# CederGroupHub/sparse-lm

Measured on AMD Instinct MI355X. Metric: fits/sec over 50-alpha Lasso path at n=100k p=5k, higher is better.
Workload: dtype f64

## Files before the change

include/slm_engine.h:

```cpp
#ifndef SLM_ENGINE_H
#define SLM_ENGINE_H

#include <stddef.h>
#include <stdint.h>

#ifdef __cplusplus
extern "C" {
#endif

#define SLM_ABI_VERSION 22

typedef enum slm_status {
  SLM_OK = 0,
  SLM_ERR_BAD_ARG = 1,
  SLM_ERR_OOM = 2,
  SLM_ERR_HIP = 3,
  SLM_ERR_NO_DEVICE = 4,
  SLM_ERR_COMM = 5,
  SLM_ERR_NOT_CONVERGED = 6,
  SLM_ERR_NON_FINITE = 7,
  SLM_ERR_UNSUPPORTED = 8
} slm_status;

typedef struct slm_engine slm_engine;
typedef struct slm_dataset slm_dataset;
// ... 186 lines not shown
int slm_solve_constrained(slm_dataset* ds, const double* a, const double* A, int32_t m, const double* lo, const double* hi,
                          const slm_solve_opts* opts, double tol_inner, int32_t max_sweeps, const double* beta0, int32_t warm,
                          double* beta_out, double* lambda_out, slm_point_info* info);

int slm_dataset_covariance(slm_dataset* ds, const double* row_weight, int64_t n_eff);
int slm_dataset_covariance_folds(slm_dataset* ds, const double* const* row_weights, const int64_t* n_effs, int32_t count);
int slm_dataset_covariance_folds_begin(slm_dataset* ds, const double* const* row_weights, const int64_t* n_effs, int32_t count,
                                       int32_t* started_out);
int slm_dataset_covariance_folds_finish(slm_dataset* ds);
int slm_dataset_covariance_count(slm_dataset* ds, int32_t* count_out);
int slm_dataset_covariance_clear(slm_dataset* ds);
int slm_dataset_covariance_download(slm_dataset* ds, int32_t index, double* G_out, double* c_out, double scalars_out[4]);

int slm_dataset_read_ceiling(slm_dataset* ds, int32_t reps, double* gbs_out, double* ms_out);

int slm_dataset_model_gram(slm_dataset* ds, double* G_out);
int slm_dataset_set_replicated(slm_dataset* ds, int32_t replicated);

#define SLM_COMM_ID_BYTES 128
int slm_comm_unique_id(uint8_t id_out[SLM_COMM_ID_BYTES]);
int slm_comm_init(slm_engine* eng, int32_t rank, int32_t n_ranks,
                  const uint8_t id[SLM_COMM_ID_BYTES]);
int slm_comm_info(slm_engine* eng, int32_t* rank_out, int32_t* n_ranks_out);
int slm_comm_collectives(slm_engine* eng, int64_t* count_out);
int slm_comm_all_reduce_probe(slm_engine* eng, int64_t count, int32_t reps, double* us_out);
int slm_comm_init_local(slm_engine** engines, int32_t n_ranks, double timeout_s);
int slm_dataset_set_global_rows(slm_dataset* ds, int64_t n_global);
int slm_comm_destroy(slm_engine* eng);

#ifdef __cplusplus
// ... 4 lines not shown
```

sparse-lm_amd/csrc/data_kernels.hpp:

```cpp
#pragma once
#include <hip/hip_runtime.h>
#include <stdint.h>

#include "grad_kernel.hpp"
#include "tail_kernels.hpp"

namespace slm {

static __global__ __launch_bounds__(256) void transpose_f2c_kernel(const double* __restrict__ src, int64_t n,
                                                            int64_t p, double* __restrict__ dst,
                                                            int64_t ld) {
  __shared__ double tile[32][33];
  const int tx = threadIdx.x & 31, ty = threadIdx.x >> 5;
  const int64_t i0 = (int64_t)blockIdx.x * 32, j0 = (int64_t)blockIdx.y * 32;
  for (int k = ty; k < 32; k += 8) {
    const int64_t i = i0 + tx, j = j0 + k;
    tile[k][tx] = (i < n && j < p) ? src[j * n + i] : 0.0;
  }
  __syncthreads();
  for (int k = ty; k < 32; k += 8) {
    const int64_t i = i0 + k, j = j0 + tx;
    if (i < n && j < p) dst[i * ld + j] = tile[tx][k];
  }
}

static __global__ __launch_bounds__(256) void tile_columns_kernel(const double* __restrict__ X, int64_t n, int64_t ld,
                                                           double* __restrict__ XT) {
  __shared__ double tile[32][33];
  const int tx = threadIdx.x & 31, ty = threadIdx.x >> 5;
  const int64_t i0 = (int64_t)blockIdx.x * 32, j0 = (int64_t)blockIdx.y * 32;
  for (int k = ty; k < 32; k += 8) {
    const int64_t i = i0 + k, j = j0 + tx;
    tile[k][tx] = (i < n && j < ld) ? X[i * ld + j] : 0.0;
  }
  __syncthreads();
  for (int k = ty; k < 32; k += 8) {
    const int64_t j = j0 + k;
    if (j < ld) XT[((int64_t)blockIdx.x * ld + j) * 32 + tx] = tile[tx][k];
  }
}

template <int U, bool NT, bool RR = false>
__global__ __launch_bounds__(256) void read_stream_kernel(const double* __restrict__ src, int64_t count2 ,
                                                          double* __restrict__ sink) {
  const d2* p = reinterpret_cast<const d2*>(src);
  const int64_t per = (count2 + gridDim.x - 1) / gridDim.x;
  const int64_t lo = RR ? (int64_t)blockIdx.x * (U * 256) : (int64_t)blockIdx.x * per;
  const int64_t hi = RR ? count2 : (lo + per < count2 ? lo + per : count2);
  const int64_t step = RR ? (int64_t)gridDim.x * (U * 256) : (int64_t)U * 256;
  double a0 = 0.0, a1 = 0.0;
  int64_t i = lo + threadIdx.x;
  for (; i + (int64_t)(U - 1) * 256 < hi; i += step) {
    d2 v[U];
#pragma unroll
// ... 199 lines not shown
```

sparse-lm_amd/csrc/engine.hip:

```cpp
#include "engine_internal.hpp"

static thread_local std::string g_last_error;

int fail(int code, const char* fmt, ...) {
  char buf[1024];
  va_list ap;
  va_start(ap, fmt);
  vsnprintf(buf, sizeof(buf), fmt, ap);
  va_end(ap);
  g_last_error = buf;
  return code;
}

RcclApi g_rccl;

int load_rccl() {
  if (g_rccl.lib) return SLM_OK;
  const char* names[] = {"librccl.so.1", "librccl.so", "/opt/rocm/lib/librccl.so.1"};
  void* lib = nullptr;
  for (const char* nm : names) {
    lib = dlopen(nm, RTLD_NOW | RTLD_GLOBAL);
    if (lib) break;
  }
  if (!lib) return fail(SLM_ERR_COMM, "cannot load librccl: %s", dlerror());
// ... 239 lines not shown
}

static void dataset_free(slm_dataset* ds) {
  if (!ds) return;
  dfree(ds->X); dfree(ds->y); dfree(ds->rw); dfree(ds->yzero); dfree(ds->rw_lanes); dfree(ds->rvec);
  dfree(ds->order); dfree(ds->gid); dfree(ds->gstart);
  dfree(ds->partial); dfree(ds->loss_partial); dfree(ds->R);
  dfree(ds->g); dfree(ds->z); dfree(ds->beta); dfree(ds->zprev); dfree(ds->gprev);
  dfree(ds->u); dfree(ds->gscale); dfree(ds->a0); dfree(ds->b0); dfree(ds->d0);
  dfree(ds->lambda); dfree(ds->dctl);
  dfree(ds->pts); dfree(ds->betas_out); dfree(ds->gn_out); dfree(ds->infos);
  dfree(ds->ws_idx); dfree(ds->ws_pos); dfree(ds->ws_gs); dfree(ds->ws_gl);
  dfree(ds->ws_score); dfree(ds->ws_XW); dfree(ds->ws_part); dfree(ds->ws_G); dfree(ds->ws_Gx); dfree(ds->XT); dfree(ds->ws_owner);
  dfree(ds->ws_nt); dfree(ds->stop_words); dfree(ds->sse_Z); dfree(ds->sse_part); dfree(ds->split_state);
  dfree(ds->cons_state); dfree(ds->cons_buf);
  dfree(ds->colnorm); dfree(ds->lt_dR); dfree(ds->lt_d2); dfree(ds->lt_part); dfree(ds->lt_cols); dfree(ds->lt_stamp);
  cov_pending_drop(ds);
  ds->cov.clear();
  ds->cov_all_hold.reset();
  ds->cov_all = nullptr;
  dfree(ds->cov_Z); dfree(ds->cov_fp); dfree(ds->cov_partial);
  mg_free(ds);
  if (ds->h_split) (void)hipHostFree(ds->h_split);
  if (ds->hctl) (void)hipHostFree(ds->hctl);
  if (ds->h_small_out) (void)hipHostFree(ds->h_small_out);
  if (ds->h_vec) (void)hipHostFree(ds->h_vec);
  if (ds->h_stage) (void)hipHostFree(ds->h_stage);
  if (ds->h_pts) (void)hipHostFree(ds->h_pts);
  for (auto& e : ds->ev)
    if (e) (void)hipEventDestroy(e);
// ... 561 lines not shown
```

sparse-lm_amd/csrc/engine_internal.hpp:

```cpp
#pragma once
#include <hip/hip_runtime.h>

#include <dlfcn.h>
#include <stdarg.h>
#include <stdio.h>
#include <stdlib.h>
#include <string.h>

#include <algorithm>
#include <cmath>
#include <chrono>
#include <condition_variable>
#include <memory>
#include <mutex>
#include <numeric>
#include <string>
#include <vector>

#include "../../include/slm_engine.h"
#include "host_logic.hpp"
#include "data_kernels.hpp"
#include "grad_kernel.hpp"
#include "tail_kernels.hpp"
#include "ws_kernels.hpp"
// ... 182 lines not shown
  double* cov_Z = nullptr;
  double* cov_partial = nullptr;
  int cov_partial_sets = 0;
  size_t partial_elems = 0;
  double* cov_fp = nullptr;
  double* split_state = nullptr;
  double* h_split = nullptr;
  double* cons_state = nullptr;
  double* cons_buf = nullptr;
  size_t cons_buf_doubles = 0;
  double* stop_words = nullptr;
  double* XT = nullptr;
  bool XT_ready = false, XT_failed = false;
  double* colnorm = nullptr;
  bool colnorm_ready = false;
  double *lt_dR = nullptr, *lt_d2 = nullptr, *lt_part = nullptr;
  int32_t *lt_cols = nullptr, *lt_stamp = nullptr;
  struct MgEntry {
    float* G = nullptr;
    double fp1 = 0.0, fp2 = 0.0, n_eff = 0.0;
    bool own = false;
  };
  std::vector<MgEntry> mg;
  double* mg_vec = nullptr;
  double* mg_Z = nullptr;
  bool mg_failed = false;
  double mg_build_ms = 0.0;
  int ws_sets = 0;
  const GradKernel* gk[SLM_MAX_LANES] = {};
  int nblk[SLM_MAX_LANES] = {};
// ... 54 lines not shown

struct LaneSetup {
  int B = 1;
  const double* rw = nullptr;
  int64_t rw_stride = 0;
  double n_eff[SLM_MAX_CELLS] = {};
};
LaneSetup default_lanes(slm_dataset* ds, int B);
int enqueue_gradient(slm_dataset* ds, const LaneSetup& ls, const double* y, const int* done, hipEvent_t ev_start, hipEvent_t ev_stop,
                     int64_t n_rows = 0, const int* skip = nullptr, GradNames* names = nullptr);
int enqueue_gradient_split(const slm_host::Knobs& kn, slm_dataset* ds, const LaneSetup& ls, const double* y, const int* done, const PathCtl* ctl, const WsArgs* wa,
                           hipEvent_t ev_start, hipEvent_t ev_stop, int64_t n_rows = 0, bool unit_bracket = false, const int* skip = nullptr,
                           GradNames* names = nullptr);
bool split_usable(const slm_host::Knobs& kn, slm_dataset* ds);
int ensure_xt(const slm_host::Knobs& kn, slm_dataset* ds);
int check_launch();
void launch_rowdot(const slm_host::Knobs& kn, slm_dataset* ds, const SplitKernel* sk, int nblk, int B, SplitArgs& a, hipStream_t s,
                  const char** name = nullptr);
int enqueue_gradient_cov(slm_dataset* ds, int B, const int* entry_of, const int* done, hipEvent_t ev_start, hipEvent_t ev_stop,
                         const PathCtl* ctl = nullptr, const WsArgs* wa = nullptr, GradNames* names = nullptr);
void launch_tail(const TailArgs& ta, hipStream_t s);
int64_t sketch_rows(int64_t n);
int power_iteration(const slm_host::Knobs& kn, slm_dataset* ds, const LaneSetup& ls_in, double* L_out , int iters, int64_t n_rows = 0);
int estimate_lipschitz(const slm_host::Knobs& kn, slm_dataset* ds, double* L_out, int iters);
int allow_big_lds(const void* fn, int device);
static const int kProfStride = 3;
static const int kPowerItersSolve = 2;
int cov_fingerprints(slm_dataset* ds, const double* const* w, int count, double* out );
int cov_find(const slm_dataset* ds, double fp1, double fp2, double n_eff);
void cov_pending_drop(slm_dataset* ds);
// ... 9 lines not shown
```

sparse-lm_amd/csrc/engine_path.hip:

```cpp
#include "engine_internal.hpp"

static int ws_policy(const slm_host::Knobs& kn, const slm_dataset* ds, uint32_t flags) {
  if (ds->max_group > WS_KCAP / 2 || ds->n < 4) return 0;
  if (kn.ws == 0 || (flags & SLM_FLAG_NO_WORKING_SET)) return 0;
  const bool big = (double)ds->n * (double)ds->ld >= 67108864.0;
  return (big || (flags & SLM_FLAG_WORKING_SET) || kn.ws == 1) ? 2 : 1;
}

static bool small_ok(const slm_host::Knobs& kn, const slm_dataset* ds, uint32_t flags) {
  if (!(flags & SLM_FLAG_ON_CHIP)) return false;
  if (flags & (SLM_FLAG_NO_RESTART | SLM_FLAG_PROFILE | SLM_FLAG_FISTA_ONLY | SLM_FLAG_WORKING_SET | SLM_FLAG_NO_WORKING_SET))
    return false;
  if (!kn.on_chip) return false;
  return ds->p <= SM_PMAX && (double)ds->n * (double)ds->ld <= 131072.0 && !row_sharded(ds);
}
static bool split_possible(const slm_dataset* ds) {
  return ds->sk != nullptr && (ds->sk->rowdot != nullptr || !ds->XT_failed);
}
static int max_lanes_for(const slm_host::Knobs& kn, const slm_dataset* ds, uint32_t flags) {
  if (small_ok(kn, ds, flags)) return ds->lane_cap;
  if ((ws_policy(kn, ds, flags) == 2 || (double)ds->n * (double)ds->ld >= 67108864.0) && split_possible(ds)) {
    if (ws_policy(kn, ds, flags) == 2 && !row_sharded(ds) && ds->sk->rowdot != nullptr && !ds->XT_failed)
      return kMaxLanes;
    return SPLIT_LANES;
// ... 908 lines not shown
    for (int l = 0; l < B; ++l) {
      int64_t mine = lanes[l].n_points;
      if (shared_path && interleave) mine = slm_host::interleaved_points(slm_host::LaneWalk{h[l].pt_lo, h[l].n_points, h[l].stride, h[l].tail_pt});
      most = std::max<int64_t>(most, mine);
    }
    expected = 1 + most;
    planned_end = expected;
  }
  {
    bool cold = true;
    for (int l = 0; l < B; ++l) cold = cold && lanes[l].beta0 == nullptr;
    if (cold && shared_path && use_ws && !ws_late && !sharded && !cov_on && split && !any_rw && !ds->rw &&
        !custom_scale && expected > 0 && o.max_iter >= 4 && !(o.flags & SLM_FLAG_FISTA_ONLY) && kn.sample_start) {
      const int64_t least = kn.sample_min_rows;
      if (n >= least) n_sample = n / kn.sample_div;
    }
  }
  mg_forced = kn.mg == 2;
  mg_cap = slm_host::model_gram_cap(ld, 3.0e9, kMgEntries);
  mg_ok = use_ws && split && (big_x || mg_forced) && !sharded && !cov_on && !(o.flags & SLM_FLAG_NO_MODEL_GRAM) &&
                     (size_t)ds->lane_cap >= (size_t)kMaxLanes && ws_n_sets <= mg_cap && mg_possible(kn, ds);
  if (mg_ok && mg_forced) expected = 0;
  if (mg_ok && !mg_forced && !ds->mg.empty()) {
    bool all = ws_n_sets > 0;
    for (int st = 0; st < ws_n_sets && all; ++st) {
      const int l = ws_set_lane[st];
      all = lanes[l].row_weight == nullptr;
      const double ne = ls.n_eff[l] > 0 ? ls.n_eff[l] : (double)ds->n_global;
      bool have = false;
      for (const auto& e : ds->mg) have = have || (e.own && e.n_eff == ne);
// ... 643 lines not shown
```

sparse-lm_amd/csrc/engine_solve.hip:

```cpp
#include "engine_internal.hpp"

#define SLM_GK(W, C, R, B) {W, C, R, B, 0, grad_fused_kernel<W, C, R, B>, "grad_fused_kernel<" #W "," #C "," #R "," #B ">"}
#define SLM_RK(W, C, B, D) {W, C, 1, B, D, grad_ring_kernel<W, C, B, D>, "grad_ring_kernel<" #W "," #C "," #B "," #D ">"}
static const GradKernel kGradRing[] = {
    SLM_RK(8, 1, 1, 3), SLM_RK(8, 2, 1, 3), SLM_RK(8, 3, 1, 3), SLM_RK(8, 4, 1, 3), SLM_RK(8, 5, 1, 2),
    SLM_RK(8, 1, 2, 3), SLM_RK(8, 2, 2, 3), SLM_RK(8, 3, 2, 3), SLM_RK(8, 4, 2, 3), SLM_RK(8, 5, 2, 2),
    SLM_RK(8, 1, 3, 3), SLM_RK(8, 2, 3, 3), SLM_RK(8, 3, 3, 3), SLM_RK(8, 4, 3, 3), SLM_RK(8, 5, 3, 2),
    SLM_RK(8, 1, 4, 3), SLM_RK(8, 2, 4, 3), SLM_RK(8, 3, 4, 3), SLM_RK(8, 4, 4, 3), SLM_RK(8, 5, 4, 2),
    SLM_RK(8, 1, 5, 3), SLM_RK(8, 2, 5, 3), SLM_RK(8, 3, 5, 3), SLM_RK(8, 4, 5, 3),
    SLM_RK(8, 1, 6, 3), SLM_RK(8, 2, 6, 3), SLM_RK(8, 3, 6, 3),
};
static const GradKernel kGradDefault[] = {
    SLM_GK(1, 1, 4, 1), SLM_GK(2, 1, 4, 1), SLM_GK(4, 1, 4, 1), SLM_GK(8, 1, 4, 1), SLM_GK(8, 2, 4, 1),
    SLM_GK(8, 3, 4, 1), SLM_GK(8, 4, 2, 1), SLM_GK(8, 5, 2, 1), SLM_GK(8, 6, 2, 1), SLM_GK(8, 8, 2, 1),
    SLM_GK(8, 10, 1, 1),
    SLM_GK(1, 1, 4, 2), SLM_GK(2, 1, 4, 2), SLM_GK(4, 1, 4, 2), SLM_GK(8, 1, 4, 2), SLM_GK(8, 2, 4, 2),
    SLM_GK(8, 3, 4, 2), SLM_GK(8, 4, 2, 2), SLM_GK(8, 5, 2, 2), SLM_GK(8, 6, 2, 2), SLM_GK(8, 8, 1, 2),
    SLM_GK(1, 1, 4, 3), SLM_GK(2, 1, 4, 3), SLM_GK(4, 1, 4, 3), SLM_GK(8, 1, 4, 3), SLM_GK(8, 2, 4, 3),
    SLM_GK(8, 3, 4, 3), SLM_GK(8, 4, 2, 3), SLM_GK(8, 5, 2, 3), SLM_GK(8, 6, 1, 3),
    SLM_GK(1, 1, 4, 4), SLM_GK(2, 1, 4, 4), SLM_GK(4, 1, 4, 4), SLM_GK(8, 1, 4, 4), SLM_GK(8, 2, 4, 4),
    SLM_GK(8, 3, 2, 4), SLM_GK(8, 4, 2, 4), SLM_GK(8, 5, 1, 4),
};
static const GradKernel kGradExtra[] = {
    SLM_GK(8, 5, 1, 1), SLM_GK(8, 5, 3, 1), SLM_GK(8, 5, 4, 1), SLM_GK(8, 4, 4, 1), SLM_GK(8, 6, 1, 1),
// ... 16 lines not shown
  return &kSplitAnyWidth;
}

int xtr_max_row_blocks(int cus, int64_t ld) {
  return slm_host::xtr_row_blocks_most(cus, ld, XTR_CB);
}
int launch_xtr(const slm_host::Knobs& kn, int cus, SplitArgs& a, hipStream_t s, bool sample, const char** name) {
  double per_cu = kn.xtr_wgs_per_cu;
  const bool wide = a.lane_slots > SPLIT_LANES;
  if (wide) per_cu = 1.0;
  const slm_host::XtrGrid g = slm_host::xtr_grid(a.n, a.ld, XTR_CB, (int64_t)(xtr_max_row_blocks(cus, a.ld) * per_cu / 2.0));
  const int xb = g.xb, yb = g.yb;
  a.xrows = g.rows;
  const int extra = wide ? a.n_lanes - SPLIT_LANES : 0;
  const char* nm;
  if (wide && extra >= 1 && extra <= 2) {
    if (sample) { hipLaunchKernelGGL(xtr18_sample_kernel, dim3(xb, yb), dim3(XTR_WAVES * 64), 0, s, a); nm = "xtr18_sample_kernel"; }
    else { hipLaunchKernelGGL(xtr18_mfma_kernel, dim3(xb, yb), dim3(XTR_WAVES * 64), 0, s, a); nm = "xtr18_mfma_kernel"; }
  } else if (wide && extra >= 3 && extra <= 4) {
    if (sample) { hipLaunchKernelGGL(xtr20_sample_kernel, dim3(xb, yb), dim3(XTR_WAVES * 64), 0, s, a); nm = "xtr20_sample_kernel"; }
    else { hipLaunchKernelGGL(xtr20_mfma_kernel, dim3(xb, yb), dim3(XTR_WAVES * 64), 0, s, a); nm = "xtr20_mfma_kernel"; }
  } else if (wide) {
    if (sample) { hipLaunchKernelGGL(xtr32_sample_kernel, dim3(xb, yb), dim3(XTR_WAVES * 64), 0, s, a); nm = "xtr32_sample_kernel"; }
    else { hipLaunchKernelGGL(xtr32_mfma_kernel, dim3(xb, yb), dim3(XTR_WAVES * 64), 0, s, a); nm = "xtr32_mfma_kernel"; }
  } else {
    if (sample) { hipLaunchKernelGGL(xtr_sample_kernel, dim3(xb, yb), dim3(XTR_WAVES * 64), 0, s, a); nm = "xtr_sample_kernel"; }
    else { hipLaunchKernelGGL(xtr_mfma_kernel, dim3(xb, yb), dim3(XTR_WAVES * 64), 0, s, a); nm = "xtr_mfma_kernel"; }
  }
  if (name) *name = nm;
  return yb;
}
// ... 148 lines not shown
  const int64_t nr = n_rows > 0 ? n_rows : ds->n;
  a.n = nr; a.ld = ds->ld; a.rows_base = nr / nblk; a.rows_rem = nr % nblk;
  a.p2 = (int)(ds->ld / 2);
  a.n_lanes = ls.B;
  const bool unit = ev_start != nullptr && unit_bracket;
  if (unit) HIP_TRY(hipEventRecord(ev_start, s));
  launch_rowdot(kn, ds, sk, nblk, ls.B, a, s, names ? &names->resid : nullptr);
  if (wa && ctl) {
    const char* nm;
    if (kn.resid_vec && halves == 1) { hipLaunchKernelGGL(sk->resid, dim3(nblk), dim3(256), 0, s, a); nm = "resid_ws_kernel<16>"; }
    else if (halves == 2) { hipLaunchKernelGGL(resid32_mfma_kernel, dim3(nblk, 1), dim3(RM_WAVES * 64), 0, s, a); nm = "resid32_mfma_kernel"; }
    else { hipLaunchKernelGGL(resid_mfma_kernel, dim3(nblk, halves), dim3(RM_WAVES * 64), 0, s, a); nm = "resid_mfma_kernel"; }
    if (names) names->ws_resid = nm;
  }
  if (ev_start && !unit) HIP_TRY(hipEventRecord(ev_start, s));
  const int xblk = launch_xtr(kn, ds->eng->cus, a, s, n_rows > 0 && ctl != nullptr,
                              names ? &names->product : nullptr);
  if (ev_stop) HIP_TRY(hipEventRecord(ev_stop, s));
  ReduceArgs ra;
  ra.partial = ds->partial;
  ra.loss_partial = ds->loss_partial;
  ra.g = ds->g;
  ra.done = done;
  ra.nblk = xblk;
  ra.nblk_loss = nblk;
  ra.skip = skip;
  ra.n_lanes = a.lane_slots;
  ra.ld = ds->ld;
  for (int l = 0; l < kMaxLanes; ++l) {
    const double ne = ls.n_eff[l] > 0 ? ls.n_eff[l] : (double)ds->n_global;
    ra.scale[l] = 1.0 / ne;
    ra.loss_scale[l] = 0.5 / ne;
// ... 180 lines not shown
  HIP_TRY(hipMemsetAsync(ds->z, 0, sizeof(double) * ld, s));
  LaneSetup ls = default_lanes(ds, 1);
  ls.n_eff[0] = sums[0];
  SLM_TRY(enqueue_gradient(ds, ls, ds->yzero, nullptr, nullptr, nullptr));
  HIP_TRY(hipMemsetAsync(ds->yzero, 0, sizeof(double) * n, s));
  const int cblocks = ds->eng->cus * 8;
  hipLaunchKernelGGL(center_kernel, dim3(cblocks), dim3(256), 0, s, ds->X, ds->y, n, p, ld, ds->g, ymean);
  SLM_TRY(check_launch());
  if (x_mean_out) HIP_TRY(hipMemcpyAsync(x_mean_out, ds->g, sizeof(double) * p, hipMemcpyDeviceToHost, s));
  HIP_TRY(hipStreamSynchronize(s));
  if (y_mean_out) *y_mean_out = ymean;
  ds->L_valid = false;
  ds->sketch_valid = false;
  ds->carry_valid = false;
  ds->XT_ready = false;
  mg_invalidate(ds);
  return SLM_OK;
}

template <typename Launch>
static int timed_launches(hipStream_t s, int reps, double* ms_out, Launch launch) {
  hipEvent_t e0, e1;
  HIP_TRY(hipEventCreate(&e0));
  HIP_TRY(hipEventCreate(&e1));
  HIP_TRY(hipEventRecord(e0, s));
  int rc = SLM_OK;
  for (int r = 0; r < reps && rc == SLM_OK; ++r) rc = launch();
  HIP_TRY(hipEventRecord(e1, s));
  HIP_TRY(hipEventSynchronize(e1));
  float ms = 0.f;
// ... 295 lines not shown
    ds->XT_ready = true;
    ds->colnorm_ready = false;
    const dim3 grid((unsigned)row_tiles, (unsigned)((ld + 31) / 32));
    hipLaunchKernelGGL(tile_columns_kernel, grid, dim3(256), 0, s, (const double*)ds->X, n, ld, ds->XT);
  }
  if (ds->XT && ds->XT_ready && !ds->colnorm_ready && !ds->rw && !row_sharded(ds) && kn.light_pass) {
    if (!ds->colnorm && pool_malloc((void**)&ds->colnorm, sizeof(double) * (size_t)ld) != hipSuccess) {
      (void)hipGetLastError();
      ds->colnorm = nullptr;
    }
    if (ds->colnorm) {
      hipLaunchKernelGGL(colnorm_kernel, dim3((unsigned)((ld + 7) / 8)), dim3(256), 0, s, (const double*)ds->XT, n, ld, 1.0 / (double)ds->n_global,
                         ds->colnorm);
      ds->colnorm_ready = true;
    }
  }
  return SLM_OK;
}

extern "C" int slm_eval_sse_sparse(slm_dataset* ds, const int32_t* cols, int32_t n_cols, const double* Zs,
                                   int32_t m, const double* row_weight, double* sse_out) {
  if (!ds || !cols || !Zs || !sse_out) return fail(SLM_ERR_BAD_ARG, "NULL argument");
  if (m <= 0 || n_cols <= 0) return fail(SLM_ERR_BAD_ARG, "m and n_cols must be positive");
  if (n_cols > WS_KCAP) return fail(SLM_ERR_UNSUPPORTED, "more than %d columns: use slm_eval_sse", WS_KCAP);
  for (int k = 0; k < n_cols; ++k)
    if (cols[k] < 0 || cols[k] >= ds->p) return fail(SLM_ERR_BAD_ARG, "cols[%d] = %d outside [0, p)", k, cols[k]);
  slm_engine* eng = ds->eng;
  HIP_TRY(hipSetDevice(eng->device));
  hipStream_t s = eng->stream;
  const int64_t n = ds->n;
// ... 279 lines not shown
```

sparse-lm_amd/csrc/host_logic.hpp:

```cpp
#pragma once
#include <stddef.h>
#include <math.h>
#include <stdint.h>
#include <stdio.h>
#include <stdlib.h>

#include <algorithm>
#include <utility>
#include <vector>

#if defined(__HIPCC__)
#define SLM_HD __host__ __device__
#else
#define SLM_HD
#endif

namespace slm_host {

struct PoolLedger {
  struct Idle { int dev; size_t bytes; void* block; };
  struct Live { void* block; int dev; size_t bytes; };
  std::vector<Idle> idle;
  std::vector<Live> live;
  size_t idle_bytes = 0;
// ... 197 lines not shown
  bool carry = true;
  bool ws_carry = true;
  bool eval_fused = false;
  double ws_theta = 0.85;
  int ws_append = 48;
  int ws_kinit = 0;
  int ws_bb = 1;
  int ws_one_solver = 0;
  bool hard_callwide = false;
  int ws_miss_factor = 4;
  int ws_miss_div = 8;
  double ws_fill = 0.0;
  bool sample_start = true;
  int64_t sample_min_rows = 65536;
  int sample_div = 4;
  int mg = -1;
  bool handover = true;
  bool light_pass = true;
  bool lag_handover = true;
  bool gram_owner = true;
  double device_pool_gb = -1.0;
  bool allow_any_arch = false;
  int trace = 0;
  bool trace_poll = false;

  template <typename Get>
  static Knobs from(Get get) {
    Knobs k;
    auto text = [&](const char* name) -> const char* { return get(name); };
    auto is_set = [&](const char* name) { return text(name) != nullptr; };
// ... 26 lines not shown
    if (const char* e = text("SLM_WS_THETA")) {
      const double v = atof(e);
      if (v > 0.0 && v <= 1.0) k.ws_theta = v;
    }
    as_int("SLM_WS_APPEND", 1, 512, &k.ws_append);
    as_int("SLM_WS_KINIT", 16, 512, &k.ws_kinit);
    if (const char* e = text("SLM_WS_BB")) k.ws_bb = atoi(e) != 0;
    if (const char* e = text("SLM_WS_ONE_SOLVER")) k.ws_one_solver = atoi(e) != 0;
    k.hard_callwide = is_set("SLM_HARD_CALLWIDE");
    as_int("SLM_WS_MISS_FACTOR", 1, 8, &k.ws_miss_factor);
    as_int("SLM_WS_MISS_DIV", 1, 4096, &k.ws_miss_div);
    if (const char* e = text("SLM_WS_FILL")) k.ws_fill = std::max(0.1, std::min(1.0, atof(e)));
    k.sample_start = !is_set("SLM_NO_SAMPLE_START");
    if (const char* e = text("SLM_SAMPLE_START_MIN_ROWS")) k.sample_min_rows = std::max<int64_t>(64, atoll(e));
    as_int("SLM_SAMPLE_DIV", 1, 64, &k.sample_div);
    if (const char c = first("SLM_MG")) k.mg = c == '0' ? 0 : (c == '2' ? 2 : -1);
    k.handover = !is_set("SLM_NO_HANDOVER");
    k.light_pass = !is_set("SLM_NO_LIGHT_PASS");
    k.gram_owner = !is_set("SLM_NO_GRAM_OWNER");
    k.lag_handover = !is_set("SLM_NO_LAG_HANDOVER");
    if (const char* e = text("SLM_DEVICE_POOL_GB")) k.device_pool_gb = std::max(0.0, atof(e));
    k.allow_any_arch = is_set("SLM_ALLOW_ANY_ARCH");
    if (const char c = first("SLM_TRACE")) k.trace = (c >= '1' && c <= '3') ? c - '0' : 1;
    k.trace_poll = is_set("SLM_TRACE_POLL");
    return k;
  }
};

}
```

sparse-lm_amd/csrc/split_kernels.hpp:

```cpp
#pragma once
#include <hip/hip_runtime.h>
#include <stdint.h>

#include "grad_kernel.hpp"
#include "tail_kernels.hpp"
#include "ws_kernels.hpp"

namespace slm {

constexpr int SPLIT_LANES = 16;
constexpr int SPLIT_RSTRIDE = 16;
constexpr int SPLIT_HALVES = SLM_MAX_LANES / SPLIT_LANES;
static_assert(SLM_MAX_LANES % SPLIT_LANES == 0 && SPLIT_HALVES >= 1 && SPLIT_HALVES <= 2, "one or two halves of sixteen lanes");
constexpr int ROWDOT_LANES = 5;

struct SplitArgs {
  const double* X;
  const double* y;
  const double* rw;
  int64_t rw_stride;
  const double* z;
  double* R;
  double* partial;
  double* loss_partial;
  const int* done;
  const PathCtl* ctl;
  const double* XW;
  const int32_t* idx;
  const WsCtl* ws;
  int64_t n, ld, rows_base, rows_rem;
  int p2;
  int n_lanes;
  int lane0;
  int xrows;
  int xrows_ws;
  const double* XT;
  int lane_slots;
  int64_t r_plane;
  const int* skip;
};
__device__ __forceinline__ bool split_off(const SplitArgs& a) {
  return (a.done != nullptr && *a.done != 0) || (a.skip != nullptr && *a.skip != 0);
}
__device__ __forceinline__ int split_slots(const SplitArgs& a) { return a.lane_slots > 0 ? a.lane_slots : SPLIT_LANES; }

__device__ __forceinline__ void split_masks(const SplitArgs& a, unsigned& live, unsigned& on_ws, int half = 0) {
  const int l = threadIdx.x & 63;
  const int L = SPLIT_LANES * half + l;
  int lv = 0, sp = 0;
  if (l < SPLIT_LANES && L < a.n_lanes) {
    if (a.ctl == nullptr) {
      lv = 1;
    } else {
      const int dn = a.ctl[L].done, id = a.ctl[L].idle, zs = a.ctl[L].zsup;
// ... 411 lines not shown
            if (col < ld) out[col] = acc[h][2 * c + e][r];
          }
    }
  }
}

static __global__ __launch_bounds__(XTR_WAVES * 64, 2) void xtr_mfma_kernel(SplitArgs a) { xtr_mfma_body<1>(a); }
static __global__ __launch_bounds__(XTR_WAVES * 64, 1) void xtr32_mfma_kernel(SplitArgs a) { xtr_mfma_body<2>(a); }
static __global__ __launch_bounds__(XTR_WAVES * 64, 2) void xtr_sample_kernel(SplitArgs a) { xtr_mfma_body<1>(a); }
static __global__ __launch_bounds__(XTR_WAVES * 64, 1) void xtr32_sample_kernel(SplitArgs a) { xtr_mfma_body<2>(a); }
static __global__ __launch_bounds__(XTR_WAVES * 64, 1) void xtr18_mfma_kernel(SplitArgs a) { xtr_mfma_body<1, 2>(a); }
static __global__ __launch_bounds__(XTR_WAVES * 64, 1) void xtr20_mfma_kernel(SplitArgs a) { xtr_mfma_body<1, 4>(a); }
static __global__ __launch_bounds__(XTR_WAVES * 64, 1) void xtr18_sample_kernel(SplitArgs a) { xtr_mfma_body<1, 2>(a); }
static __global__ __launch_bounds__(XTR_WAVES * 64, 1) void xtr20_sample_kernel(SplitArgs a) { xtr_mfma_body<1, 4>(a); }

constexpr int XZ_WAVES = 4;
constexpr int XZ_T = 4;

template <int NT, int H, int E = 0>
__device__ __forceinline__ void rowdot_step(const double* xt0, int64_t ld, const double* const (&zp)[H],
                                            const double* const (&zpe)[E > 0 ? E : 1], int g_n, double* mine, double* pe) {
  constexpr int EE = E > 0 ? E : 1;
  slm_d4 acc[H][NT][2];
#pragma unroll
  for (int h = 0; h < H; ++h)
#pragma unroll
    for (int t = 0; t < NT; ++t) acc[h][t][0] = acc[h][t][1] = slm_d4{0.0, 0.0, 0.0, 0.0};
  d2 ex[EE][NT];
#pragma unroll
  for (int e = 0; e < EE; ++e)
// ... 414 lines not shown
```

sparse-lm_amd/sparselm_amd/_engine.py:

```python

from __future__ import annotations

import ctypes as C
import os
import sys
import threading
import weakref

import numpy as np

_LIB_NAME = "libslm_hip.so"
_LIB_DIR = os.path.join(os.path.dirname(os.path.abspath(__file__)), "_lib")

SLM_OK = 0
SLM_ERR_BAD_ARG = 1
SLM_ERR_OOM = 2
SLM_ERR_HIP = 3
SLM_ERR_NO_DEVICE = 4
SLM_ERR_COMM = 5
SLM_ERR_NOT_CONVERGED = 6
SLM_ERR_NON_FINITE = 7
SLM_ERR_UNSUPPORTED = 8

FLAG_NO_RESTART = 1
FLAG_PROFILE = 2
FLAG_COLD_START = 4
FLAG_FRESH_L = 8
FLAG_FISTA_ONLY = 16
FLAG_WORKING_SET = 32
FLAG_NO_WORKING_SET = 64
FLAG_ON_CHIP = 128
FLAG_COVARIANCE = 256
FLAG_PROFILE_UNIT = 1024
FLAG_NO_MODEL_GRAM = 512

COMM_ID_BYTES = 128
ABI_VERSION = 22

ABI_SYMBOLS = (
    "slm_abi_version",
    "slm_last_error",
    "slm_device_count",
    "slm_host_alloc",
    "slm_host_free",
    "slm_engine_create",
    "slm_engine_destroy",
    "slm_engine_synchronize",
    "slm_reload_knobs",
    "slm_engine_device_info",
    "slm_dataset_create",
    "slm_dataset_create_device",
    "slm_dataset_create_synthetic",
# ... 19 lines not shown
    "slm_solve_path",
    "slm_solve_lanes",
    "slm_solve_lanes_reweighted",
    "slm_solve_path_lanes",
    "slm_solve_standardized_sgl",
    "slm_solve_constrained",
    "slm_dataset_covariance",
    "slm_dataset_covariance_folds",
    "slm_dataset_covariance_folds_begin",
    "slm_dataset_covariance_folds_finish",
    "slm_dataset_covariance_count",
    "slm_dataset_covariance_clear",
    "slm_dataset_covariance_download",
    "slm_dataset_model_gram",
    "slm_dataset_read_ceiling",
    "slm_dataset_set_replicated",
    "slm_comm_unique_id",
    "slm_comm_init",
    "slm_comm_info",
    "slm_comm_collectives",
    "slm_comm_all_reduce_probe",
    "slm_comm_init_local",
    "slm_dataset_set_global_rows",
    "slm_comm_destroy",
)


class EngineError(RuntimeError):
    """HIP / RCCL / device failure reported by the engine."""

# ... 202 lines not shown
            "slm_solve_lanes_reweighted": [vp, P(_Lane), P(_Reweight), i32, P(_SolveOpts), P(_SolveStats), P(i32)],
            "slm_solve_path_lanes": [
                vp, P(_PenaltyStruct), P(_PathPoint), i32, i32, P(_SolveOpts), vp, vp, vp, P(_PointInfo), P(_SolveStats),
            ],
            "slm_solve_standardized_sgl": [vp, vp, vp, P(_SolveOpts), dbl, i32, vp, i32, vp, vp, P(_PointInfo)],
            "slm_solve_constrained": [vp, vp, vp, i32, vp, vp, P(_SolveOpts), dbl, i32, vp, i32, vp, vp, P(_PointInfo)],
            "slm_dataset_covariance": [vp, vp, i64],
            "slm_dataset_covariance_folds": [vp, vp, vp, i32],
            "slm_dataset_covariance_folds_begin": [vp, vp, vp, i32, P(i32)],
            "slm_dataset_covariance_folds_finish": [vp],
            "slm_dataset_covariance_count": [vp, P(i32)],
            "slm_dataset_covariance_clear": [vp],
            "slm_dataset_covariance_download": [vp, i32, vp, vp, vp],
            "slm_dataset_model_gram": [vp, vp],
            "slm_dataset_read_ceiling": [vp, i32, P(dbl), P(dbl)],
            "slm_dataset_set_replicated": [vp, i32],
            "slm_comm_unique_id": [vp],
            "slm_comm_init": [vp, i32, i32, vp],
            "slm_comm_info": [vp, P(i32), P(i32)],
            "slm_comm_collectives": [vp, P(i64)],
            "slm_comm_all_reduce_probe": [vp, i64, i32, P(dbl)],
            "slm_comm_init_local": [P(vp), i32, dbl],
            "slm_dataset_set_global_rows": [vp, i64],
            "slm_comm_destroy": [vp],
        }
        for name, argtypes in sigs.items():
            fn = getattr(lib, name)
            fn.argtypes = argtypes
            fn.restype = C.c_int
        _lib = lib
# ... 641 lines not shown
        _check(self._lib.slm_dataset_covariance_folds_finish(self._h))

    def covariance_download(self, index: int):
        G = np.empty((self.p, self.p))
        c = np.empty(self.p)
        sc = np.empty(4)
        _check(self._lib.slm_dataset_covariance_download(self._h, int(index), _ptr(G), _ptr(c), _ptr(sc)))
        return G, c, {"yy": float(sc[0]), "n_eff": float(sc[1]), "fingerprint": (float(sc[2]), float(sc[3]))}

    def read_ceiling(self, reps: int = 5) -> tuple[float, float]:
        _sync_knobs()
        gbs, ms = C.c_double(), C.c_double()
        _check(self._lib.slm_dataset_read_ceiling(self._h, int(reps), C.byref(gbs), C.byref(ms)))
        return float(gbs.value), float(ms.value)

    def model_gram(self, download: bool = False):
        _sync_knobs()
        ld = (self.p + 15) // 16 * 16
        G = np.empty((ld, ld)) if download else None
        _check(self._lib.slm_dataset_model_gram(self._h, _ptr(G) if download else None))
        return G

    def set_replicated(self, replicated: bool = True):
        _check(self._lib.slm_dataset_set_replicated(self._h, int(bool(replicated))))

    def covariance_clear(self):
        _check(self._lib.slm_dataset_covariance_clear(self._h))

    def covariance_count(self) -> int:
        out = C.c_int32()
# ... 157 lines not shown
```

Measured before the change: 17070.

## Add float32 copy of X for sample-phase screening X^T R products

Builds a float32 copy of the design matrix once per dataset, along with per-column rounding-error statistics, and uses it in new screening kernels for the sampled-row X^T R products. The kernels upcast to f64 before the MFMA, so the aim is to halve the bytes read from X during the bandwidth-bound sample start. The cost is extra device memory, a one-time build pass with a host sync, and approximation error in the screening gradients that the later full f64 passes have to correct.

```diff
diff --git a/include/slm_engine.h b/include/slm_engine.h
--- a/include/slm_engine.h
+++ b/include/slm_engine.h
@@ -8,7 +8,7 @@
 extern "C" {
 #endif
 
-#define SLM_ABI_VERSION 22
+#define SLM_ABI_VERSION 23
 
 typedef enum slm_status {
   SLM_OK = 0,
@@ -225,6 +225,8 @@
 
 int slm_dataset_read_ceiling(slm_dataset* ds, int32_t reps, double* gbs_out, double* ms_out);
 
+int slm_dataset_screen_copy(slm_dataset* ds, int32_t* state_out, int64_t* launches_out, double* err_out);
+
 int slm_dataset_model_gram(slm_dataset* ds, double* G_out);
 int slm_dataset_set_replicated(slm_dataset* ds, int32_t replicated);
 
diff --git a/sparse-lm_amd/csrc/data_kernels.hpp b/sparse-lm_amd/csrc/data_kernels.hpp
--- a/sparse-lm_amd/csrc/data_kernels.hpp
+++ b/sparse-lm_amd/csrc/data_kernels.hpp
@@ -38,6 +38,44 @@
     const int64_t j = j0 + k;
     if (j < ld) XT[((int64_t)blockIdx.x * ld + j) * 32 + tx] = tile[tx][k];
   }
+}
+
+constexpr int X32_ROW_BLOCKS = 256;
+static __global__ __launch_bounds__(256) void x32_build_kernel(const double* __restrict__ X, int64_t n, int64_t ld, float* __restrict__ X32,
+                                                              double* __restrict__ err_part, int* __restrict__ bad) {
+  const int64_t j = (int64_t)blockIdx.x * 256 + threadIdx.x;
+  if (j >= ld) return;
+  const int64_t nb = gridDim.y, b = blockIdx.y;
+  const int64_t base = n / nb, rem = n % nb;
+  const int64_t r0 = b * base + (b < rem ? b : rem), r1 = r0 + base + (b < rem ? 1 : 0);
+  double acc = 0.0;
+  bool any_bad = false;
+  auto one = [&](int64_t i, double x) {
+    const float v = (float)x;
+    X32[i * ld + j] = v;
+    any_bad = any_bad || !(fabsf(v) <= 3.402823466e+38f);
+    const double d = x - (double)v;
+    acc = __builtin_fma(d, d, acc);
+  };
+  int64_t i = r0;
+  for (; i + 8 <= r1; i += 8) {
+    double x[8];
+#pragma unroll
+    for (int u = 0; u < 8; ++u) x[u] = X[(i + u) * ld + j];
+#pragma unroll
+    for (int u = 0; u < 8; ++u) one(i + u, x[u]);
+  }
+  for (; i < r1; ++i) one(i, X[i * ld + j]);
+  err_part[b * ld + j] = acc;
+  if (any_bad) *bad = 1;
+}
+static __global__ __launch_bounds__(256) void x32_error_kernel(const double* __restrict__ err_part, int nblk, int64_t ld, double inv_n,
+                                                              double* __restrict__ err) {
+  const int64_t j = (int64_t)blockIdx.x * 256 + threadIdx.x;
+  if (j >= ld) return;
+  double s = 0.0;
+  for (int b = 0; b < nblk; ++b) s += err_part[(int64_t)b * ld + j];
+  err[j] = sqrt(s * inv_n);
 }
 
 template <int U, bool NT, bool RR = false>
diff --git a/sparse-lm_amd/csrc/engine.hip b/sparse-lm_amd/csrc/engine.hip
--- a/sparse-lm_amd/csrc/engine.hip
+++ b/sparse-lm_amd/csrc/engine.hip
@@ -277,6 +277,7 @@
   dfree(ds->ws_score); dfree(ds->ws_XW); dfree(ds->ws_part); dfree(ds->ws_G); dfree(ds->ws_Gx); dfree(ds->XT); dfree(ds->ws_owner);
   dfree(ds->ws_nt); dfree(ds->stop_words); dfree(ds->sse_Z); dfree(ds->sse_part); dfree(ds->split_state);
   dfree(ds->cons_state); dfree(ds->cons_buf);
+  dfree(ds->X32); dfree(ds->x32_err);
   dfree(ds->colnorm); dfree(ds->lt_dR); dfree(ds->lt_d2); dfree(ds->lt_part); dfree(ds->lt_cols); dfree(ds->lt_stamp);
   cov_pending_drop(ds);
   ds->cov.clear();
diff --git a/sparse-lm_amd/csrc/engine_internal.hpp b/sparse-lm_amd/csrc/engine_internal.hpp
--- a/sparse-lm_amd/csrc/engine_internal.hpp
+++ b/sparse-lm_amd/csrc/engine_internal.hpp
@@ -220,6 +220,10 @@
   bool XT_ready = false, XT_failed = false;
   double* colnorm = nullptr;
   bool colnorm_ready = false;
+  float* X32 = nullptr;
+  double* x32_err = nullptr;
+  bool x32_ready = false, x32_refused = false;
+  int64_t x32_launches = 0;
   double *lt_dR = nullptr, *lt_d2 = nullptr, *lt_part = nullptr;
   int32_t *lt_cols = nullptr, *lt_stamp = nullptr;
   struct MgEntry {
@@ -304,6 +308,7 @@
                            GradNames* names = nullptr);
 bool split_usable(const slm_host::Knobs& kn, slm_dataset* ds);
 int ensure_xt(const slm_host::Knobs& kn, slm_dataset* ds);
+bool ensure_x32(const slm_host::Knobs& kn, slm_dataset* ds);
 int check_launch();
 void launch_rowdot(const slm_host::Knobs& kn, slm_dataset* ds, const SplitKernel* sk, int nblk, int B, SplitArgs& a, hipStream_t s,
                   const char** name = nullptr);
diff --git a/sparse-lm_amd/csrc/engine_path.hip b/sparse-lm_amd/csrc/engine_path.hip
--- a/sparse-lm_amd/csrc/engine_path.hip
+++ b/sparse-lm_amd/csrc/engine_path.hip
@@ -946,6 +946,7 @@
         !custom_scale && expected > 0 && o.max_iter >= 4 && !(o.flags & SLM_FLAG_FISTA_ONLY) && kn.sample_start) {
       const int64_t least = kn.sample_min_rows;
       if (n >= least) n_sample = n / kn.sample_div;
+      if (n_sample > 0 && B <= SPLIT_LANES + 4) (void)ensure_x32(kn, ds);
     }
   }
   mg_forced = kn.mg == 2;
diff --git a/sparse-lm_amd/csrc/engine_solve.hip b/sparse-lm_amd/csrc/engine_solve.hip
--- a/sparse-lm_amd/csrc/engine_solve.hip
+++ b/sparse-lm_amd/csrc/engine_solve.hip
@@ -54,7 +54,11 @@
   a.xrows = g.rows;
   const int extra = wide ? a.n_lanes - SPLIT_LANES : 0;
   const char* nm;
-  if (wide && extra >= 1 && extra <= 2) {
+  const bool screen = sample && a.X32 != nullptr && (!wide || (extra >= 1 && extra <= 4));
+  if (screen && !wide) { hipLaunchKernelGGL(xtr_screen_sample_kernel, dim3(xb, yb), dim3(XTR_WAVES * 64), 0, s, a); nm = "xtr_screen_sample_kernel"; }
+  else if (screen && extra <= 2) { hipLaunchKernelGGL(xtr18_screen_sample_kernel, dim3(xb, yb), dim3(XTR_WAVES * 64), 0, s, a); nm = "xtr18_screen_sample_kernel"; }
+  else if (screen) { hipLaunchKernelGGL(xtr20_screen_sample_kernel, dim3(xb, yb), dim3(XTR_WAVES * 64), 0, s, a); nm = "xtr20_screen_sample_kernel"; }
+  else if (wide && extra >= 1 && extra <= 2) {
     if (sample) { hipLaunchKernelGGL(xtr18_sample_kernel, dim3(xb, yb), dim3(XTR_WAVES * 64), 0, s, a); nm = "xtr18_sample_kernel"; }
     else { hipLaunchKernelGGL(xtr18_mfma_kernel, dim3(xb, yb), dim3(XTR_WAVES * 64), 0, s, a); nm = "xtr18_mfma_kernel"; }
   } else if (wide && extra >= 3 && extra <= 4) {
@@ -233,8 +237,12 @@
     if (names) names->ws_resid = nm;
   }
   if (ev_start && !unit) HIP_TRY(hipEventRecord(ev_start, s));
-  const int xblk = launch_xtr(kn, ds->eng->cus, a, s, n_rows > 0 && ctl != nullptr,
-                              names ? &names->product : nullptr);
+  const bool sample = n_rows > 0 && ctl != nullptr;
+  if (sample && !ls.rw && ls.B <= SPLIT_LANES + 4 && ensure_x32(kn, ds)) {
+    a.X32 = ds->X32;
+    ds->x32_launches += 1;
+  }
+  const int xblk = launch_xtr(kn, ds->eng->cus, a, s, sample, names ? &names->product : nullptr);
   if (ev_stop) HIP_TRY(hipEventRecord(ev_stop, s));
   ReduceArgs ra;
   ra.partial = ds->partial;
@@ -445,6 +453,8 @@
   ds->sketch_valid = false;
   ds->carry_valid = false;
   ds->XT_ready = false;
+  ds->x32_ready = false;
+  ds->x32_refused = false;
   mg_invalidate(ds);
   return SLM_OK;
 }
@@ -770,6 +780,50 @@
                          ds->colnorm);
       ds->colnorm_ready = true;
     }
+  }
+  return SLM_OK;
+}
+
+bool ensure_x32(const slm_host::Knobs& kn, slm_dataset* ds) {
+  if (!kn.screen_pass || ds->rw || row_sharded(ds) || ds->x32_refused) return false;
+  if (ds->n * ds->ld < kn.screen_min_entries) return false;
+  if (ds->X32 && ds->x32_ready) return true;
+  hipStream_t s = ds->eng->stream;
+  const int64_t n = ds->n, ld = ds->ld;
+  const int nblk = (int)std::min<int64_t>(X32_ROW_BLOCKS, n);
+  double* part = nullptr;
+  int* bad = nullptr;
+  auto refuse = [&]() {
+    (void)hipGetLastError();
+    dfree(part); dfree(bad); dfree(ds->X32); dfree(ds->x32_err);
+    ds->x32_ready = false;
+    ds->x32_refused = true;
+    return false;
+  };
+  if (!ds->X32 && pool_malloc((void**)&ds->X32, sizeof(float) * (size_t)n * (size_t)ld) != hipSuccess) { ds->X32 = nullptr; return refuse(); }
+  if (!ds->x32_err && pool_malloc((void**)&ds->x32_err, sizeof(double) * (size_t)ld) != hipSuccess) { ds->x32_err = nullptr; return refuse(); }
+  if (pool_malloc((void**)&part, sizeof(double) * (size_t)nblk * (size_t)ld) != hipSuccess) { part = nullptr; return refuse(); }
+  if (pool_malloc((void**)&bad, sizeof(int)) != hipSuccess) { bad = nullptr; return refuse(); }
+  int bad_host = 1;
+  if (hipMemsetAsync(bad, 0, sizeof(int), s) != hipSuccess) return refuse();
+  hipLaunchKernelGGL(x32_build_kernel, dim3((unsigned)((ld + 255) / 256), (unsigned)nblk), dim3(256), 0, s, (const double*)ds->X, n, ld, ds->X32, part, bad);
+  hipLaunchKernelGGL(x32_error_kernel, dim3((unsigned)((ld + 255) / 256)), dim3(256), 0, s, (const double*)part, nblk, ld, 1.0 / (double)n, ds->x32_err);
+  if (hipMemcpyAsync(&bad_host, bad, sizeof(int), hipMemcpyDeviceToHost, s) != hipSuccess || hipStreamSynchronize(s) != hipSuccess) return refuse();
+  if (bad_host != 0) return refuse();
+  dfree(part); dfree(bad);
+  ds->x32_ready = true;
+  return true;
+}
+
+extern "C" int slm_dataset_screen_copy(slm_dataset* ds, int32_t* state_out, int64_t* launches_out, double* err_out) {
+  if (!ds) return fail(SLM_ERR_BAD_ARG, "NULL argument");
+  HIP_TRY(hipSetDevice(ds->eng->device));
+  const bool have = ds->X32 != nullptr && ds->x32_ready;
+  if (state_out) *state_out = have ? 1 : (ds->x32_refused ? -1 : 0);
+  if (launches_out) *launches_out = ds->x32_launches;
+  if (err_out && have) {
+    HIP_TRY(hipMemcpyAsync(err_out, ds->x32_err, sizeof(double) * (size_t)ds->p, hipMemcpyDeviceToHost, ds->eng->stream));
+    HIP_TRY(hipStreamSynchronize(ds->eng->stream));
   }
   return SLM_OK;
 }
diff --git a/sparse-lm_amd/csrc/host_logic.hpp b/sparse-lm_amd/csrc/host_logic.hpp
--- a/sparse-lm_amd/csrc/host_logic.hpp
+++ b/sparse-lm_amd/csrc/host_logic.hpp
@@ -235,6 +235,8 @@
   bool sample_start = true;
   int64_t sample_min_rows = 65536;
   int sample_div = 4;
+  bool screen_pass = true;
+  int64_t screen_min_entries = int64_t(1) << 26;
   int mg = -1;
   bool handover = true;
   bool light_pass = true;
@@ -291,6 +293,8 @@
     k.sample_start = !is_set("SLM_NO_SAMPLE_START");
     if (const char* e = text("SLM_SAMPLE_START_MIN_ROWS")) k.sample_min_rows = std::max<int64_t>(64, atoll(e));
     as_int("SLM_SAMPLE_DIV", 1, 64, &k.sample_div);
+    k.screen_pass = !is_set("SLM_NO_SCREEN_PASS");
+    if (const char* e = text("SLM_SCREEN_MIN_ENTRIES")) k.screen_min_entries = std::max<int64_t>(0, atoll(e));
     if (const char c = first("SLM_MG")) k.mg = c == '0' ? 0 : (c == '2' ? 2 : -1);
     k.handover = !is_set("SLM_NO_HANDOVER");
     k.light_pass = !is_set("SLM_NO_LIGHT_PASS");
diff --git a/sparse-lm_amd/csrc/split_kernels.hpp b/sparse-lm_amd/csrc/split_kernels.hpp
--- a/sparse-lm_amd/csrc/split_kernels.hpp
+++ b/sparse-lm_amd/csrc/split_kernels.hpp
@@ -38,6 +38,7 @@
   int lane_slots;
   int64_t r_plane;
   const int* skip;
+  const float* X32;
 };
 __device__ __forceinline__ bool split_off(const SplitArgs& a) {
   return (a.done != nullptr && *a.done != 0) || (a.skip != nullptr && *a.skip != 0);
@@ -479,6 +480,167 @@
 static __global__ __launch_bounds__(XTR_WAVES * 64, 1) void xtr18_sample_kernel(SplitArgs a) { xtr_mfma_body<1, 2>(a); }
 static __global__ __launch_bounds__(XTR_WAVES * 64, 1) void xtr20_sample_kernel(SplitArgs a) { xtr_mfma_body<1, 4>(a); }
 
+typedef float slm_f4 __attribute__((ext_vector_type(4)));
+constexpr int XTS_U = 4;
+
+template <int E>
+__device__ __forceinline__ void xtr_screen_body(SplitArgs& a) {
+  static_assert(SPLIT_RSTRIDE == 16 && SPLIT_LANES == 16, "a row of a plane of R is the 16-wide B operand");
+  static_assert(E == 0 || E == 2 || E == 4, "extras: pairs of slots of plane 1 beside the sixteen of plane 0");
+  constexpr int E2 = E > 0 ? E / 2 : 1;
+  if (split_off(a)) return;
+  const int lane = threadIdx.x & 63;
+  const int wave = __builtin_amdgcn_readfirstlane((int)threadIdx.x >> 6);
+  int bx = (int)blockIdx.x, by = (int)blockIdx.y;
+  {
+    const int total = (int)(gridDim.x * gridDim.y), lin = bx + (int)gridDim.x * by;
+    const int xcd = lin & 7, slot = lin >> 3, base = total >> 3, rem = total & 7;
+    const int m = xcd * base + (xcd < rem ? xcd : rem) + slot;
+    bx = m % (int)gridDim.x;
+    by = m / (int)gridDim.x;
+  }
+  const int col0 = (bx * XTR_WAVES + wave) * XTR_CW;
+  const int ld = (int)a.ld;
+  if (col0 >= ld) return;
+  const int64_t r0 = (int64_t)by * a.xrows;
+  const int64_t r1 = r0 + a.xrows < a.n ? r0 + a.xrows : a.n;
+  const int kq = lane >> 4, i16 = lane & 15;
+  int coff[2];
+#pragma unroll
+  for (int c = 0; c < 2; ++c) {
+    const int col = col0 + 64 * c + 4 * i16;
+    coff[c] = col < ld - 4 ? col : ld - 4;
+  }
+  slm_d4 acc[8];
+#pragma unroll
+  for (int t = 0; t < 8; ++t) acc[t] = slm_d4{0.0, 0.0, 0.0, 0.0};
+  double ex[2 * E2][8];
+#pragma unroll
+  for (int e = 0; e < 2 * E2; ++e)
+#pragma unroll
+    for (int t = 0; t < 8; ++t) ex[e][t] = 0.0;
+  const int nb = (int)((r1 - r0) / (4 * XTS_U));
+  const float* xp = a.X32 + (r0 + kq) * a.ld;
+  const double* rp = a.R + (r0 + kq) * SPLIT_RSTRIDE + i16;
+  const double* rp1 = a.R + a.r_plane + (r0 + kq) * SPLIT_RSTRIDE;
+  slm_f4 xa[XTS_U][2], xb[XTS_U][2];
+  double ra[XTS_U], rb[XTS_U];
+  d2 ea[E2][XTS_U], eb[E2][XTS_U];
+  auto load = [&](slm_f4(&xv)[XTS_U][2], double(&rv)[XTS_U], d2(&ev)[E2][XTS_U], int b) {
+    const float* xq = xp + (int64_t)b * (4 * XTS_U) * a.ld;
+    const double* rq = rp + (int64_t)b * (4 * XTS_U) * SPLIT_RSTRIDE;
+#pragma unroll
+    for (int u = 0; u < XTS_U; ++u) {
+#pragma unroll
+      for (int c = 0; c < 2; ++c) {
+        const slm_f4* src = reinterpret_cast<const slm_f4*>(xq + (int64_t)u * 4 * a.ld + coff[c]);
+        xv[u][c] = SLM_NT_LOADS ? __builtin_nontemporal_load(src) : *src;
+      }
+      rv[u] = rq[u * 4 * SPLIT_RSTRIDE];
+      if constexpr (E > 0) {
+        const d2* eq = reinterpret_cast<const d2*>(rp1 + ((int64_t)b * (4 * XTS_U) + u * 4) * SPLIT_RSTRIDE);
+#pragma unroll
+        for (int q = 0; q < E2; ++q) ev[q][u] = eq[q];
+      }
+    }
+  };
+  auto step = [&](const slm_f4(&x)[2], double rv, const d2(&ev)[E2]) {
+#pragma unroll
+    for (int c = 0; c < 2; ++c)
+#pragma unroll
+      for (int m = 0; m < 4; ++m) {
+        const double xd = (double)x[c][m];
+        acc[4 * c + m] = __builtin_amdgcn_mfma_f64_16x16x4f64(xd, rv, acc[4 * c + m], 0, 0, 0);
+        if constexpr (E > 0) {
+#pragma unroll
+          for (int q = 0; q < E2; ++q) {
+            ex[2 * q][4 * c + m] = __builtin_fma(xd, ev[q].x, ex[2 * q][4 * c + m]);
+            ex[2 * q + 1][4 * c + m] = __builtin_fma(xd, ev[q].y, ex[2 * q + 1][4 * c + m]);
+          }
+        }
+      }
+  };
+  auto compute = [&](slm_f4(&xv)[XTS_U][2], double(&rv)[XTS_U], d2(&ev)[E2][XTS_U]) {
+#pragma unroll
+    for (int u = 0; u < XTS_U; ++u) {
+      d2 eu[E2];
+#pragma unroll
+      for (int q = 0; q < E2; ++q) eu[q] = ev[q][u];
+      step(xv[u], rv[u], eu);
+    }
+  };
+  if (nb > 0) {
+    load(xa, ra, ea, 0);
+    const int pairs = (nb - 1) >> 1;
+    for (int k = 0; k < pairs; ++k) {
+      load(xb, rb, eb, 2 * k + 1);
+      compute(xa, ra, ea);
+      load(xa, ra, ea, 2 * k + 2);
+      compute(xb, rb, eb);
+    }
+    if ((nb - 1) & 1) {
+      load(xb, rb, eb, nb - 1);
+      compute(xa, ra, ea);
+      compute(xb, rb, eb);
+    } else {
+      compute(xa, ra, ea);
+    }
+  }
+  for (int64_t row = r0 + (int64_t)nb * (4 * XTS_U); row < r1; row += 4) {
+    const bool ok = row + kq < r1;
+    const int64_t rr = ok ? row + kq : r1 - 1;
+    const double rv = ok ? a.R[rr * SPLIT_RSTRIDE + i16] : 0.0;
+    slm_f4 x[2];
+#pragma unroll
+    for (int c = 0; c < 2; ++c) x[c] = *reinterpret_cast<const slm_f4*>(a.X32 + rr * a.ld + coff[c]);
+    d2 eu[E2];
+#pragma unroll
+    for (int q = 0; q < E2; ++q) eu[q] = d2{0.0, 0.0};
+    if constexpr (E > 0) {
+#pragma unroll
+      for (int q = 0; q < E2; ++q)
+        if (ok) eu[q] = reinterpret_cast<const d2*>(a.R + a.r_plane + rr * SPLIT_RSTRIDE)[q];
+    }
+    step(x, rv, eu);
+  }
+  constexpr int SLOTS = E > 0 ? 2 * SPLIT_LANES : SPLIT_LANES;
+  if constexpr (E > 0) {
+#pragma unroll
+    for (int e = 0; e < E; ++e) {
+      double* out = a.partial + ((int64_t)by * SLOTS + SPLIT_LANES + e) * a.ld;
+#pragma unroll
+      for (int c = 0; c < 2; ++c) {
+        double v[4];
+#pragma unroll
+        for (int m = 0; m < 4; ++m) {
+          v[m] = ex[e][4 * c + m];
+          v[m] += __shfl_xor(v[m], 16, 64);
+          v[m] += __shfl_xor(v[m], 32, 64);
+        }
+        const int col = col0 + 64 * c + 4 * i16;
+        if (kq == 0 && col < ld) {
+          *reinterpret_cast<d2*>(out + col) = d2{v[0], v[1]};
+          *reinterpret_cast<d2*>(out + col + 2) = d2{v[2], v[3]};
+        }
+      }
+    }
+  }
+  double* out = a.partial + ((int64_t)by * SLOTS + i16) * a.ld;
+#pragma unroll
+  for (int c = 0; c < 2; ++c)
+#pragma unroll
+    for (int m = 0; m < 4; ++m)
+#pragma unroll
+      for (int r = 0; r < 4; ++r) {
+        const int col = col0 + 64 * c + 4 * (kq + 4 * r) + m;
+        if (col < ld) out[col] = acc[4 * c + m][r];
+      }
+}
+
+static __global__ __launch_bounds__(XTR_WAVES * 64, 2) void xtr_screen_sample_kernel(SplitArgs a) { xtr_screen_body<0>(a); }
+static __global__ __launch_bounds__(XTR_WAVES * 64, 1) void xtr18_screen_sample_kernel(SplitArgs a) { xtr_screen_body<2>(a); }
+static __global__ __launch_bounds__(XTR_WAVES * 64, 1) void xtr20_screen_sample_kernel(SplitArgs a) { xtr_screen_body<4>(a); }
+
 constexpr int XZ_WAVES = 4;
 constexpr int XZ_T = 4;
 
diff --git a/sparse-lm_amd/sparselm_amd/_engine.py b/sparse-lm_amd/sparselm_amd/_engine.py
--- a/sparse-lm_amd/sparselm_amd/_engine.py
+++ b/sparse-lm_amd/sparselm_amd/_engine.py
@@ -35,7 +35,7 @@
 FLAG_NO_MODEL_GRAM = 512
 
 COMM_ID_BYTES = 128
-ABI_VERSION = 22
+ABI_VERSION = 23
 
 ABI_SYMBOLS = (
     "slm_abi_version",
@@ -85,6 +85,7 @@
     "slm_dataset_covariance_download",
     "slm_dataset_model_gram",
     "slm_dataset_read_ceiling",
+    "slm_dataset_screen_copy",
     "slm_dataset_set_replicated",
     "slm_comm_unique_id",
     "slm_comm_init",
@@ -317,6 +318,7 @@
             "slm_dataset_covariance_download": [vp, i32, vp, vp, vp],
             "slm_dataset_model_gram": [vp, vp],
             "slm_dataset_read_ceiling": [vp, i32, P(dbl), P(dbl)],
+            "slm_dataset_screen_copy": [vp, P(i32), P(i64), vp],
             "slm_dataset_set_replicated": [vp, i32],
             "slm_comm_unique_id": [vp],
             "slm_comm_init": [vp, i32, i32, vp],
@@ -988,6 +990,12 @@
         _check(self._lib.slm_dataset_read_ceiling(self._h, int(reps), C.byref(gbs), C.byref(ms)))
         return float(gbs.value), float(ms.value)
 
+    def screen_copy(self, errors: bool = False):
+        state, launches = C.c_int32(), C.c_int64()
+        err = np.zeros(self.p) if errors else None
+        _check(self._lib.slm_dataset_screen_copy(self._h, C.byref(state), C.byref(launches), _ptr(err) if errors else None))
+        return {"state": int(state.value), "launches": int(launches.value), "err": err if errors and state.value == 1 else None}
+
     def model_gram(self, download: bool = False):
         _sync_knobs()
         ld = (self.p + 15) // 16 * 16
```

Result: no change. 17030 (-0.2%).
